# WarmCongee/SDUMC

Measured on AMD Instinct MI355X. Metric: train samples/sec at MOSEI feature shapes (two-stream forward + 6-term loss + backward + Adam), higher is better.
Workload: dtype f32

## Files before the change

### include/sdumc_hip.h

```cpp
#ifndef SDUMC_HIP_H
#define SDUMC_HIP_H

#include <stddef.h>
#include <stdint.h>

#ifdef __cplusplus
extern "C" {
#endif

#define SDUMC_OK 0
#define SDUMC_EINVAL (-1)
#define SDUMC_ELAUNCH (-2)
#define SDUMC_ENOMEM (-3)

#define SDUMC_MAX_GROUPS 8
#define SDUMC_D 256
#define SDUMC_H 128
#define SDUMC_NQ 7
#define SDUMC_RNC_DIM 64
#define SDUMC_N_SITES 35

typedef struct sdumc_dropout {
  uint32_t enabled;
  uint32_t site;
// ... 203 lines not shown
  size_t workspace_bytes;
  float* dq_sum;
  float* dout_masked;
} sdumc_attnpool_bwd_t;

size_t sdumc_attnpool_bwd_workspace_bytes(int32_t V, int32_t T, int32_t nq);
int sdumc_attnpool_bwd(const sdumc_attnpool_bwd_t* p, void* stream);
typedef struct sdumc_umca {
  sdumc_attnpool a;
  const float* w_in;
  const float* b_in;
  const void* x_p3;
  const void* w_in_p3f;
} sdumc_umca;
int sdumc_umca_fwd(const sdumc_umca* p, void* stream);

int sdumc_attnpool_fwd_multi(const sdumc_attnpool* sites, int32_t n, void* stream);
int sdumc_attnpool_bwd_multi(const sdumc_attnpool_bwd_t* sites, int32_t n, void* stream);
int sdumc_attnpool_set_v2_(int on);


int sdumc_relu_drop_bwd(const float* dy, const float* y, float scale, float* dz, int64_t n, void* stream);

size_t sdumc_colsum_workspace_bytes(int64_t rows, int32_t cols);
int sdumc_colsum(const float* a, int64_t rows, int32_t cols, int32_t lda, float* out, int32_t accumulate,
                 float* workspace, void* stream);

int sdumc_add_n(const float* const* xs, int32_t k, float* y, int64_t n, void* stream);

typedef struct sdumc_dropsum {
// ... 372 lines not shown
```

### sdumc_amd/_lib.py

```python
import ctypes as C
import os

_HERE = os.path.dirname(os.path.abspath(__file__))
LIB_PATH = os.environ.get("SDUMC_LIB") or os.path.join(_HERE, "csrc", "libsdumc_hip.so")

MAX_GROUPS = 8
D, H, NQ, RNC_DIM, N_SITES = 256, 128, 7, 64, 35
NT, NN, TN = 0, 1, 2
ACT_NONE, ACT_RELU, ACT_TANH = 0, 1, 2

c_float_p = C.c_void_p


class Dropout(C.Structure):
    _fields_ = [("enabled", C.c_uint32), ("site", C.c_uint32), ("threshold", C.c_uint32), ("scale", C.c_float),
                ("rows", C.c_uint32), ("width", C.c_uint32), ("samples", C.c_uint32), ("sample0", C.c_uint32),
                ("call0", C.c_uint32), ("stream0", C.c_uint32), ("seed_lo", C.c_uint32), ("seed_hi", C.c_uint32),
                ("dev_state", C.c_void_p), ("bits", C.c_void_p)]


class Gemm(C.Structure):
    _fields_ = [("layout", C.c_int32), ("M", C.c_int32), ("N", C.c_int32), ("K", C.c_int32),
                ("groups", C.c_int32),
                ("A", C.c_void_p * MAX_GROUPS), ("B", C.c_void_p * MAX_GROUPS),
# ... 266 lines not shown
    "sdumc_p3_join": (C.c_int, [C.c_void_p, C.c_int64, C.c_void_p, C.c_int64, C.c_int64, C.c_int32, C.c_void_p]),
    "sdumc_gemm_b1_workspace_bytes": (C.c_size_t, [C.POINTER(GemmB1)]),
    "sdumc_gemm_b1_nt": (C.c_int, [C.POINTER(GemmB1), C.c_void_p]),
    "sdumc_b1_frag_multi": (C.c_int, [C.c_void_p, C.c_void_p, C.POINTER(C.c_int64), C.POINTER(C.c_int64), C.POINTER(C.c_int32),
                                      C.POINTER(C.c_int32), C.c_int, C.c_void_p]),
    "sdumc_gemm_rows256": (C.c_int, [C.POINTER(RowsProblem), C.c_int32, C.c_void_p]),
    "sdumc_gemm_rows256_bf16": (C.c_int, [C.POINTER(RowsProblem), C.c_int32, C.c_void_p]),
    "sdumc_attnpool_fwd_workspace_bytes": (C.c_size_t, [C.c_int32, C.c_int32, C.c_int32]),
    "sdumc_attnpool_fwd": (C.c_int, [C.POINTER(AttnPool), C.c_void_p]),
    "sdumc_attnpool_fwd_workspace_bytes_dim": (C.c_size_t, [C.c_int32, C.c_int32, C.c_int32, C.c_int32]),
    "sdumc_attnpool_bwd_workspace_bytes_dim": (C.c_size_t, [C.c_int32, C.c_int32, C.c_int32, C.c_int32]),
    "sdumc_attnpool_bwd_workspace_bytes": (C.c_size_t, [C.c_int32, C.c_int32, C.c_int32]),
    "sdumc_attnpool_bwd": (C.c_int, [C.POINTER(AttnPoolBwd), C.c_void_p]),
    "sdumc_attnpool_fwd_multi": (C.c_int, [C.POINTER(AttnPool), C.c_int32, C.c_void_p]),
    "sdumc_umca_fwd": (C.c_int, [C.POINTER(Umca), C.c_void_p]),
    "sdumc_attnpool_bwd_multi": (C.c_int, [C.POINTER(AttnPoolBwd), C.c_int32, C.c_void_p]),
    "sdumc_relu_drop_bwd": (C.c_int, [C.c_void_p, C.c_void_p, C.c_float, C.c_void_p, C.c_int64, C.c_void_p]),
    "sdumc_colsum_workspace_bytes": (C.c_size_t, [C.c_int64, C.c_int32]),
    "sdumc_colsum": (C.c_int, [C.c_void_p, C.c_int64, C.c_int32, C.c_int32, C.c_void_p, C.c_int32, C.c_void_p, C.c_void_p]),
    "sdumc_add_n": (C.c_int, [C.POINTER(C.c_void_p), C.c_int32, C.c_void_p, C.c_int64, C.c_void_p]),
    "sdumc_dropsum_bwd": (C.c_int, [C.POINTER(DropSum), C.c_void_p]),
    "sdumc_fusion_fwd": (C.c_int, [C.c_void_p, C.c_void_p, C.c_void_p, C.c_int32, C.c_void_p]),
    "sdumc_fusion_bwd": (C.c_int, [C.c_void_p, C.c_void_p, C.c_void_p, C.c_void_p, C.c_void_p, C.c_int32, C.c_void_p]),
    "sdumc_hweight_fwd": (C.c_int, [C.c_void_p, C.c_void_p, C.c_void_p, C.c_int32, C.c_void_p]),
    "sdumc_hweight_bwd": (C.c_int, [C.c_void_p, C.c_void_p, C.c_void_p, C.c_void_p, C.c_void_p, C.c_void_p, C.c_int32, C.c_float, C.c_void_p]),
    "sdumc_zpool_fwd": (C.c_int, [C.c_void_p, C.c_void_p, C.c_void_p, C.c_int32, C.c_void_p]),
    "sdumc_zpool_bwd": (C.c_int, [C.c_void_p, C.c_void_p, C.c_void_p, C.c_void_p, C.c_void_p, C.c_int32, C.c_void_p]),
    "sdumc_mse_fwd_bwd": (C.c_int, [C.c_void_p, C.c_void_p, C.c_int32, C.c_float, C.c_float, C.c_void_p, C.c_void_p, C.c_void_p]),
    "sdumc_ssd_workspace_bytes": (C.c_size_t, [C.c_int64]),
    "sdumc_ssd": (C.c_int, [C.c_void_p, C.c_void_p, C.c_int64, C.c_void_p, C.c_void_p, C.c_void_p]),
# ... 153 lines not shown
```

### sdumc_amd/csrc/attn_pool.hip

```cpp
#include <type_traits>

#include "common.h"
#include "p3_loop.h"
#include <cstring>

namespace {

constexpr int D = SDUMC_D;
constexpr int MAXQ = 8;
constexpr int CH = 64;

__device__ __forceinline__ f32x4 ld4(const float* p) { return *reinterpret_cast<const f32x4*>(p); }
__device__ __forceinline__ void st4(float* p, f32x4 v) { *reinterpret_cast<f32x4*>(p) = v; }
__device__ __forceinline__ void stf_dev(float* p, float v) { __hip_atomic_store(p, v, __ATOMIC_RELAXED, __HIP_MEMORY_SCOPE_AGENT); }
__device__ __forceinline__ float ldf_dev(const float* p) { return __hip_atomic_load(p, __ATOMIC_RELAXED, __HIP_MEMORY_SCOPE_AGENT); }
__device__ __forceinline__ void st4_dev(float* p, f32x4 v) {
#pragma unroll
  for (int j = 0; j < 4; ++j) stf_dev(p + j, v[j]);
}
__device__ __forceinline__ f32x4 ld4_dev(const float* p) {
  f32x4 v;
#pragma unroll
  for (int j = 0; j < 4; ++j) v[j] = ldf_dev(p + j);
  return v;
// ... 114 lines not shown
    const size_t o = ((size_t)v * nq + i) * DD + 4 * cq;
    st4(p.pooled + o, sum);
    if (od.enabled) sum *= drop_mask4(od, (uint32_t)(v * nq + i), (uint32_t)cq);
    st4(p.out + o, sum);
  }
  float* attn = p.attn + (size_t)v * T * nq;
  for (int e = tid; e < T * nq; e += 256) {
    const int t = e / nq, i = e - t * nq;
    attn[e] = (DEV ? ldf_dev(attn + e) : attn[e]) * fac[(t / CH) * MAXQ + i];
  }
}

constexpr int UMCA_LDK = D + 4;
template <bool PHILOX, int C, bool HF = false, bool KLDS = false>
__device__ __forceinline__ void attn_fwd_partial_body(const sdumc_attnpool p, float* ws, const int nchunk, const int chunk, const int v,
                                                      const float* k_lds = nullptr, float* q_ext = nullptr, float* red_ext = nullptr) {
  constexpr int DD = D * C, LDQ = DD + 16;
  constexpr int RED = 4 * MAXQ * D > MAXQ * LDQ ? 4 * MAXQ * D : MAXQ * LDQ;
  __shared__ __attribute__((aligned(16))) float P_s[CH * MAXQ];
  float* red;
  if constexpr (KLDS) {
    red = red_ext;
  } else {
    __shared__ __attribute__((aligned(16))) float red_s[RED];
    red = red_s;
  }
  __shared__ float wstat[4][16];
  __shared__ float cstat[16];
  const int tid = threadIdx.x, lane = tid & 63, wave = tid >> 6;
  const int r16 = lane & 15, kk = lane >> 4;
  const int T = p.T, nq = p.nq;
  const int t0 = chunk * CH;
  const FwdWs w = fwd_ws(ws, p.V, nchunk, nq, DD);
  const bool fuse = p.tickets != nullptr;
  const int Tv = p.lengths ? min(T, max(1, p.lengths[v])) : T;

  float* q_s = KLDS ? q_ext : red;
  for (int e = tid; e < MAXQ * (DD / 4); e += 256) {
    const int i = e / (DD / 4), cq = e - i * (DD / 4);
    st4(q_s + i * LDQ + 4 * cq, i < nq ? ld4(p.q + (size_t)v * p.q_stride + (size_t)i * DD + 4 * cq) : f32x4{0.f, 0.f, 0.f, 0.f});
  }
  __syncthreads();
  constexpr int RB = 4;
  const DropRT xd = drop_resolve(p.x_drop);
// ... 1165 lines not shown
}
template <bool MASK>
__global__ __launch_bounds__(256, 2) void umca_fwd_kernel(const sdumc_umca u, const int nchunk) {
  extern __shared__ __attribute__((aligned(16))) char lds[];
  umca_fwd_body<MASK, false>(u, nchunk, lds);
}
template <bool MASK>
__global__ __launch_bounds__(256, 2) void umca_fwd_split_kernel(const sdumc_umca u, const int nchunk) {
  extern __shared__ __attribute__((aligned(16))) char lds[];
  umca_fwd_body<MASK, true>(u, nchunk, lds);
}

using K3P3Cfg_m = sdumc_p3::PCfg<64, 4, true, 4>;
using K3P3Cfg_n = sdumc_p3::PCfg<64, 4, false, 4>;
static_assert(K3P3Cfg_m::LDS_BYTES <= TOP_BYTES, "the P3 ring lies inside the key tile's memory");
template <bool MASK>
__global__ __launch_bounds__(256, 2) void umca_fwd_p3_kernel(const sdumc_umca u, const int nchunk) {
#if defined(__HIP_DEVICE_COMPILE__)
  using CF = std::conditional_t<MASK, K3P3Cfg_m, K3P3Cfg_n>;
  extern __shared__ __attribute__((aligned(16))) char lds[];
  const sdumc_attnpool& p = u.a;
  const int tid = threadIdx.x, lane = tid & 63;
  const int wave = __builtin_amdgcn_readfirstlane(tid >> 6);
  const int li = lane & 31, lh = lane >> 5;
  const int wn0 = wave * 64;
  const int chunk = blockIdx.x, v = blockIdx.y;
  const int T = p.T, t0 = chunk * CH, vx = v % p.x_samples;
  const __amdgpu_buffer_rsrc_t ra = __builtin_amdgcn_make_buffer_rsrc(const_cast<void*>(u.x_p3), 0,
      (int)min((size_t)p.x_samples * T * D * 6, (size_t)0xFFFFFFF0u), 0x00020000);
  const uint32_t qw = (p.x_drop.width + 3u) >> 2;
  const __amdgpu_buffer_rsrc_t rbits = __builtin_amdgcn_make_buffer_rsrc(const_cast<uint8_t*>(MASK ? p.x_drop.bits : static_cast<const uint8_t*>(u.x_p3)), 0,
      MASK ? (int)min((size_t)p.V * T * qw, (size_t)0xFFFFFFF0u) : 0, 0x00020000);
  f32x16 acc[2][2];
  sdumc_p3::p3_mainloop<CF>(lds, ra, (int64_t)D * 6, [&](int row) { return vx * T + min(t0 + row, T - 1); },
                            rbits, (int)qw, [&](int row) { return v * T + min(t0 + row, T - 1); },
                            static_cast<const char*>(u.w_in_p3f) + (size_t)(wave * 2) * (size_t)((D / 16) * sdumc_p3::FRAG_KT), (size_t)((D / 16) * sdumc_p3::FRAG_KT),
                            0, D / sdumc_p3::BK, acc);
  __syncthreads();
  const float mscale = MASK ? p.x_drop.scale : 1.f;
  float* K_s = reinterpret_cast<float*>(lds);
  float* q_s = reinterpret_cast<float*>(lds + TOP_BYTES);
  float* keys_out = const_cast<float*>(p.keys);
#pragma unroll
  for (int i = 0; i < 2; ++i)
#pragma unroll
    for (int j = 0; j < 2; ++j) {
      const int col = wn0 + 32 * j + li;
      const float bv = u.b_in[col];
#pragma unroll
      for (int e = 0; e < 16; ++e) {
        const int row = 32 * i + (e & 3) + 8 * (e >> 2) + 4 * lh;
        const float kv = fast_tanh(acc[i][j][e] * mscale + bv);
        K_s[row * UMCA_LDK + col] = kv;
        if (keys_out && t0 + row < T) keys_out[((size_t)v * T + t0 + row) * D + col] = kv;
      }
    }
  __syncthreads();
  attn_fwd_partial_body<false, 1, false, true>(p, static_cast<float*>(p.workspace), nchunk, chunk, v, K_s, q_s, K_s);
#endif
}

}

static inline uint32_t qw_of(const sdumc_dropout& d) { return (d.width + 3u) >> 2; }
extern "C" int sdumc_umca_fwd(const sdumc_umca* up, void* stream) {
  if (!up) return SDUMC_EINVAL;
  sdumc_umca u = *up;
  const sdumc_attnpool& p = u.a;
  if (p.V <= 0 || p.T <= 0 || p.nq < 1 || p.nq > MAXQ || p.x_samples <= 0) return SDUMC_EINVAL;
  if ((p.dim != 0 && p.dim != D) || p.bf16 || p.tickets) return SDUMC_EINVAL;
  if (!p.x || !p.q || !p.attn || !p.pooled || !p.out || !u.w_in || !u.b_in) return SDUMC_EINVAL;
  if (p.x_drop.enabled && !p.x_drop.bits) return SDUMC_EINVAL;
  if ((p.T + CH - 1) / CH > 4096) return SDUMC_EINVAL;
// ... 19 lines not shown
    if (p.x_drop.enabled) hipLaunchKernelGGL(sdumc_k3::umca_fwd_p3_kernel<true>, grid, blk, sdumc_k3::LDS_BYTES, st, u, nchunk);
    else hipLaunchKernelGGL(sdumc_k3::umca_fwd_p3_kernel<false>, grid, blk, sdumc_k3::LDS_BYTES, st, u, nchunk);
  } else if (sdumc_split_on_(SDUMC_SPLIT_UMCA)) {
    if (p.x_drop.enabled) hipLaunchKernelGGL(sdumc_k3::umca_fwd_split_kernel<true>, grid, blk, sdumc_k3::LDS_BYTES, st, u, nchunk);
    else hipLaunchKernelGGL(sdumc_k3::umca_fwd_split_kernel<false>, grid, blk, sdumc_k3::LDS_BYTES, st, u, nchunk);
  } else if (p.x_drop.enabled) hipLaunchKernelGGL(sdumc_k3::umca_fwd_kernel<true>, grid, blk, sdumc_k3::LDS_BYTES, st, u, nchunk);
  else hipLaunchKernelGGL(sdumc_k3::umca_fwd_kernel<false>, grid, blk, sdumc_k3::LDS_BYTES, st, u, nchunk);
  SDUMC_CHECK_LAUNCH();
  if (p.partial_only) return SDUMC_OK;
  hipLaunchKernelGGL(attn_fwd_combine_kernel, dim3(p.V), dim3(256), (size_t)nchunk * MAXQ * sizeof(float), st, p,
                     static_cast<const float*>(p.workspace), nchunk);
  SDUMC_CHECK_LAUNCH();
  return SDUMC_OK;
}

__global__ void sdumc_preload_attn_pool_kernel() {}
extern "C" int sdumc_preload_attn_pool_(void) {
  hipFuncAttributes a;
  return hipFuncGetAttributes(&a, reinterpret_cast<const void*>(&sdumc_preload_attn_pool_kernel)) == hipSuccess ? SDUMC_OK : SDUMC_ELAUNCH;
}
```

### sdumc_amd/csrc/common.h

```cpp
#pragma once
#include <hip/hip_runtime.h>
#include <stdint.h>
#include "../../include/sdumc_hip.h"

#define SDUMC_CHECK_LAUNCH()                                 \
  do {                                                       \
    if (hipGetLastError() != hipSuccess) return SDUMC_ELAUNCH; \
  } while (0)

typedef float f32x4 __attribute__((ext_vector_type(4)));
typedef float f32x16 __attribute__((ext_vector_type(16)));

static inline hipStream_t as_stream(void* s) { return (hipStream_t)s; }

#ifdef __cplusplus
#include <atomic>
#include <mutex>
struct sdumc_dev_once {
  std::mutex mu;
  std::atomic<uint64_t> done{0};
};
template <class F>
static inline int sdumc_once_per_device(sdumc_dev_once& o, F&& setup) {
  int dev = 0;
// ... 85 lines not shown
  uint32_t w[6];
};
int sdumc_dropout_bits_multi_ex_(const sdumc_dropout* d, int32_t streams, int32_t nsite, int32_t site_stride, uint8_t* const* bits,
                                 const uint32_t* tag, int32_t call_add, const struct sdumc_bits_shape* shape, void* stream);
int sdumc_bits_tag_(const sdumc_dropout* d, uint32_t* tag, int32_t call_add, const struct sdumc_bits_shape* shape, void* stream);
int sdumc_weights_to_bf16_(const float* src, void* dst, void* dst_t, const int64_t* offs, const int32_t* outs, const int32_t* ins,
                           const int32_t* want_t, int n, void* stream);
size_t sdumc_gg_slab_bytes_(int tiles);
int sdumc_gemm_rows_prepare_(void);
#define SDUMC_SPLIT_GROUP 1
#define SDUMC_SPLIT_WIDE 2
#define SDUMC_SPLIT_UMCA 4
#define SDUMC_SPLIT_ROWS 8
#define SDUMC_SPLIT_ALL 15
int sdumc_split_on_(int bit);
int sdumc_split_scope_(int mask);
int sdumc_gemm_rows256_capped_(const sdumc_rows_problem* probs, int32_t n, int32_t max_wg, void* stream);
int sdumc_gemm_rows256_bf16_capped_(const sdumc_rows_problem* probs, int32_t n, int32_t max_wg, void* stream);
int sdumc_p3_split_frag_multi_(const float* P, void* dst, const int64_t* src_off, const int64_t* dst_off, const int32_t* rows,
                               const int32_t* cols, int n, void* stream);
int sdumc_chain_transpose_(const float* src, float* dst, const int64_t* offs, const int32_t* outs, const int32_t* ins, int n,
                           void* stream);
struct sdumc_attn_layout {
  int32_t B, S;
  int32_t T[3][2];
  int64_t attn[2][3];
  int64_t total;
};
int sdumc_plan_attn_layout_(const sdumc_net_dims* d, struct sdumc_attn_layout* out);
}
// ... 99 lines not shown
```

### sdumc_amd/csrc/engine.hip

```cpp
#include <stdio.h>
#include <string.h>

#include <algorithm>
#include <atomic>
#include <map>
#include <cstdlib>
#include <cstring>
#include <mutex>
#include <string>
#include <tuple>
#include <vector>

#include "common.h"

extern "C" int sdumc_axpy2d(const float* src, int32_t ld_src, float* dst, int32_t ld_dst, int32_t rows, int32_t cols,
                            void* stream);

namespace {

constexpr int D = SDUMC_D, H = SDUMC_H, NQ = SDUMC_NQ, RD = SDUMC_RNC_DIM;

constexpr int SITE_IN[2][3] = {{0, 2, 4}, {21, 23, 25}};
constexpr int SITE_OUT[2][3] = {{1, 3, 5}, {22, 24, 26}};
constexpr int SITE_UMLP0 = 6, SITE_UMLP1 = 7;
// ... 1006 lines not shown
int p3_refresh_weights(const Ctx& c, int m) {
  const int din[3] = {c.d.da, c.d.dt, c.d.dv};
  int64_t so[3], dofs[3];
  int32_t rows[3], cols[3];
  so[0] = c.pm.frame[m].w; dofs[0] = c.pl.wp3_frame[m]; rows[0] = D; cols[0] = din[m];
  so[1] = c.pm.fra_proj[m].w; dofs[1] = c.pl.wp3_key[0][m]; rows[1] = D; cols[1] = D;
  so[2] = c.pm.ca_in[m].w; dofs[2] = c.pl.wp3_key[1][m]; rows[2] = D; cols[2] = D;
  return sdumc_p3_split_frag_multi_(c.P, wp3_ptr(c, 0), so, dofs, rows, cols, 3, c.st);
}
int feat_slot(int m, int s) { return m == 0 ? 0 : (m == 2 ? 2 : (s == 0 ? 1 : 3)); }
const int32_t* feat_map(const Ctx& c, int m, int s) { return c.io.row_map[feat_slot(m, s)]; }
int64_t feat_store_rows(const Ctx& c, int m, int s, bool both) {
  const int64_t a = c.io.store_rows[feat_slot(m, s)], b = both ? c.io.store_rows[feat_slot(m, 1)] : a;
  return (a > 0 && b > 0) ? std::max(a, b) : 0;
}
int p3_frame_proj(const Ctx& c, int m, int s, const void* feat_p3, int rows, int splitk, const void* feat2_p3 = nullptr, int rows2 = 0) {
  const int din[3] = {c.d.da, c.d.dt, c.d.dv};
  sdumc_gemm_p3 g;
  memset(&g, 0, sizeof(g));
  g.M = rows + rows2; g.N = D; g.K = din[m];
  g.A = feat_p3; g.lda = (int64_t)din[m] * 6;
  g.a_map = feat_map(c, m, s);
  g.a_map_rows = feat_store_rows(c, m, s, feat2_p3 != nullptr);
  if (feat2_p3) { g.A2 = feat2_p3; g.a2_row0 = rows; g.a2_map = feat_map(c, m, 1); }
  g.B = wp3_ptr(c, c.pl.wp3_frame[m]); g.ldb = (int64_t)(din[m] / 16) * 3072;
  g.bias = c.P + c.pm.frame[m].b;
  g.act = SDUMC_ACT_NONE;
  g.C = c.p(c.pl.x[m][s]); g.ldc = D;
  g.C_p3 = c.p(c.pl.xp3[m][s]); g.ldc_p3 = (int64_t)D * 6;
  g.splitk = splitk;
  g.workspace = c.scr;
  g.workspace_bytes = (size_t)c.pl.scratch_floats * sizeof(float);
  return sdumc_gemm_p3_nt(&g, c.st);
}
int p3_keys_fwd(const Ctx& c, int m, int k) {
  for (const Seg& sg : c.pl.segs[m]) {
    const Lin& L = k == 0 ? c.pm.fra_proj[m] : c.pm.ca_in[m];
    const sdumc_dropout dr = in_drop(c, k, m, sg.T, sg.s0, sg.row0);
    sdumc_gemm_p3 g;
    memset(&g, 0, sizeof(g));
    g.M = sg.V * sg.T; g.N = D; g.K = D;
    g.A = c.p(c.pl.xp3[m][sg.s0]); g.lda = (int64_t)D * 6;
    g.a_row_mod = sg.x_samples < sg.V ? sg.x_samples * sg.T : 0;
    if (dr.enabled) { g.a_bits = dr.bits; g.bits_qw = D / 4; g.a_scale = dr.scale; }
    g.B = wp3_ptr(c, c.pl.wp3_key[k][m]); g.ldb = (int64_t)(D / 16) * 3072;
    g.bias = c.P + L.b;
    g.act = SDUMC_ACT_TANH;
    g.C = c.p(c.pl.keys[k][m]) + sg.row0 * D; g.ldc = D;
    g.splitk = 1;
// ... 50 lines not shown
      a[n].workspace_bytes = bytes;
      ws += (bytes / sizeof(float) + 63) / 64 * 64;
      if (fra_fold(c)) fold_partial_only(c, k, order[oi], a[n]);
      ++n;
    }
  return sdumc_attnpool_fwd_multi(a, n, c.st);
}

bool k3_ok(const Ctx& c, int m) {
  static const int on = [] { const char* e = getenv("SDUMC_K3"); return e ? atoi(e) : 1; }();
  if (!on || c.h() || c.d.bf16) return false;
  for (const Seg& sg : c.pl.segs[m])
    if (sg.T < 96) return false;
  return true;
}
int umca_site(const Ctx& c, int k, int m, bool keep) {
  for (const Seg& sg : c.pl.segs[m]) {
    sdumc_umca u;
    memset(&u, 0, sizeof(u));
    u.a = attn_desc(c, k, m, sg);
    u.a.tickets = nullptr;
    if (!keep) u.a.keys = nullptr;
    u.a.workspace = c.scr;
    u.a.workspace_bytes = (size_t)c.pl.scratch_floats * sizeof(float);
    if (fra_fold(c)) fold_partial_only(c, k, m, u.a);
    const Lin& L = k == 0 ? c.pm.fra_proj[m] : c.pm.ca_in[m];
    u.w_in = c.P + L.w;
    u.b_in = c.P + L.b;
    if (p3_mode(c) && sdumc_split_on_(SDUMC_SPLIT_UMCA)) {
      u.x_p3 = c.p(c.pl.xp3[m][sg.s0]);
      u.w_in_p3f = wp3_ptr(c, c.pl.wp3_key[k][m]);
    }
    RET(sdumc_umca_fwd(&u, c.st));
  }
  return SDUMC_OK;
}

int pool_fwd(const Ctx& c, int k, int m) {
  for (const Seg& sg : c.pl.segs[m]) {
    sdumc_attnpool a = attn_desc(c, k, m, sg);
    a.workspace = c.scr;
    a.workspace_bytes = (size_t)c.pl.scratch_floats * sizeof(float);
    if (fra_fold(c)) fold_partial_only(c, k, m, a);
    RET(sdumc_attnpool_fwd(&a, c.st));
  }
  return SDUMC_OK;
}


bool use_chain(const Ctx& c) {
// ... 206 lines not shown
        if (hipEventRecord(bits_done[m], c.st) != hipSuccess) return SDUMC_ELAUNCH;
      }
    }
    if (pregen) {
      const sdumc_dropout d0 = mkdrop(c, SITE_IN[0][0], c.d.p_frame, pl.segs[0][0].T, D, 0);
      RET(sdumc_bits_tag_(&d0, reinterpret_cast<uint32_t*>(bits_set(c, 0)), 0, &shape_now, c.st));
    }
  }
  hipEvent_t fra_done[3] = {nullptr, nullptr, nullptr}, ca_done[3] = {nullptr, nullptr, nullptr};
  auto p3_frames = [&](int m) -> int {
    constexpr int p3_text_split = 4;
    RET(p3_refresh_weights(c, m));
    for (int s = 0; s < (m == 1 ? S : 1); ++s) {
      const void* fp = m == 0 ? c.io.audio_p3 : (m == 2 ? c.io.video_p3 : c.io.text_p3[s]);
      const int rows_p = B * pl.T[m][s];
      const bool few = rows_p < 8192 && din[m] >= 2048;
      if (m == 1 && S == 2 && few && rows_p % 64 == 0) {
        RET(p3_frame_proj(c, m, 0, fp, rows_p, p3_text_split, c.io.text_p3[1], B * pl.T[1][1]));
        break;
      }
      RET(p3_frame_proj(c, m, s, fp, rows_p, few ? 2 * p3_text_split : 1));
    }
    return SDUMC_OK;
  };
  for (int m = 0; m < 3; ++m) {
    c.use(LANE_OF[m]);
    if (p3_mode(c)) RET(p3_frames(m));
    if (b1_mode(c)) RET(b1_refresh_weights(c, m));
    for (int s = 0; s < (m == 1 ? S : 1) && !p3_mode(c); ++s) {
      const float* in = m == 0 ? c.io.audio : (m == 2 ? c.io.video : c.io.text[s]);
      if (b1_mode(c)) {
        const int rows_p = B * pl.T[m][s];
        if (m == 1 && S == 2 && rows_p % 64 == 0) {
          RET(b1_frame_proj(c, m, 0, in, rows_p, c.io.text[1], B * pl.T[1][1]));
          break;
        }
        RET(b1_frame_proj(c, m, s, in, rows_p));
        continue;
      }
      if (c.h()) {
        sdumc_gemm_bf16 g = GH_(SDUMC_NT, B * pl.T[m][s], D, din[m]);
        g.A[0] = in;
// ... 15 lines not shown
    }
    mark(c.st, 28 + 4 * m);
    if (bits_done[m] && hipStreamWaitEvent(c.st, bits_done[m], 0) != hipSuccess) return SDUMC_ELAUNCH;
    if (bits_with_xd) {
      for (const Seg& sg : pl.segs[m]) {
        const sdumc_dropout d = mkdrop(c, SITE_IN[0][m], c.d.p_frame, sg.T, D, sg.s0);
        uint8_t* bo[2] = {reinterpret_cast<uint8_t*>(c.p(pl.bits[0][m])) + sg.row0 * (D / 4),
                          reinterpret_cast<uint8_t*>(c.p(pl.bits[1][m])) + sg.row0 * (D / 4)};
        void* xo[2] = {c.ph(pl.xd[0][m], sg.row0 * D), c.ph(pl.xd[1][m], sg.row0 * D)};
        RET(sdumc_dropout_bits_apply_bf16(&d, sg.V / B, SITE_IN[1][m] - SITE_IN[0][m], bo, c.ph(sg.x_off), (int64_t)sg.x_samples * sg.T,
                                          xo, c.st));
      }
    }
    mark(c.st, 29 + 4 * m);
    const bool k3_site0 = k3_ok(c, m);
    constexpr int ca_own = 1;
    if (c.bg && (ca_own & (1 << m)) && LANE_OF[m] != 0 && c.multi && !c.capturing) {
      if (k3_site0) RET(umca_site(c, 0, m, true));
      else { RET(keys_gemm_fwd(c, m, 0, 1)); RET(pool_fwd(c, 0, m)); }
      fra_done[m] = next_event(c);
      if (hipEventRecord(fra_done[m], c.st) != hipSuccess) return SDUMC_ELAUNCH;
      RET(keys_gemm_fwd(c, m, 1, 2));
      ca_done[m] = next_event(c);
      if (hipEventRecord(ca_done[m], c.st) != hipSuccess) return SDUMC_ELAUNCH;
    } else if (c.bg) {
      if (k3_site0) RET(umca_site(c, 0, m, true));
      else RET(keys_gemm_fwd(c, m, 0, 1));
      RET(link(c, LANE_OF[m], 3));
      c.use(3);
      RET(keys_gemm_fwd(c, m, 1, 2));
      c.use(LANE_OF[m]);
      if (!k3_site0) RET(pool_fwd(c, 0, m));
    } else if (k3_site0) {
      RET(umca_site(c, 0, m, true));
      RET(keys_gemm_fwd(c, m, 1, 2));
    } else {
      RET(keys_gemm_fwd(c, m, 0, 2));
      RET(pool_fwd(c, 0, m));
    }
    mark(c.st, 30 + 4 * m);
  }
  mark(c.sts[3], 40);
  c.use(0);
  for (int lane = 1; lane <= 2; ++lane) {
    int m_of = -1;
    for (int m = 0; m < 3; ++m) if (LANE_OF[m] == lane && fra_done[m]) m_of = m;
    if (m_of >= 0) {
      if (hipStreamWaitEvent(c.sts[0], fra_done[m_of], 0) != hipSuccess) return SDUMC_ELAUNCH;
    } else {
// ... 1212 lines not shown
```

### sdumc_amd/csrc/gemm_f32.hip

```cpp
#include <algorithm>
#include <cstring>
#include <mutex>
#include <type_traits>
#include <vector>

#include "common.h"

namespace {

struct ProfRec {
  hipEvent_t a, b;
  int variant;
  double flops;
};
bool g_prof_on = false;
std::vector<ProfRec> g_prof;
std::mutex g_prof_mu;
constexpr int kNumVariants = 29;
const char* const kVariantName[kNumVariants] = {"gemm_nt_128x128", "gemm_nt_64x64",  "gemm_nn_128x128",
                                                "gemm_nn_64x64",   "gemm_tn_128x128", "gemm_tn_64x64",
                                                "gemm_small_nt",   "gemm_small_nn",   "gemm_small_tn",
                                                "gemm_bf16_nt_128x128", "gemm_bf16_nt_64x64",
                                                "gemm_bf16_nn_128x128", "gemm_bf16_nn_64x64",
                                                "gemm_bf16_tn_128x128", "gemm_bf16_tn_64x64",
                                                "gemm_wide_nt", "gemm_wide_tn",
                                                "gemm_bf16s_nt", "gemm_bf16s_tn",
                                                "gemm_group_tn", "gemm_group_tn_bf16",
                                                "gemm_rows256", "gemm_rows256_bf16",
                                                "gemm_wide_nt_bf16x3", "gemm_group_tn_bf16x3", "gemm_rows256_bf16x3",
                                                "gemm_p3_nt_bf16x3", "gemm_p3_nt_masked_bf16x3",
                                                "gemm_b1_nt_bf16"};

constexpr int BK = 32;
constexpr int LDK = BK + 4;
#ifndef SDUMC_GEMM_WPE128
#define SDUMC_GEMM_WPE128 2
#endif
#ifndef SDUMC_GEMM_WPE64
#define SDUMC_GEMM_WPE64 5
#endif

struct TileLoadCtx {
  const float* p;
  int ld;
  int row_mod;
  bool vec;
// ... 901 lines not shown
```

### sdumc_amd/csrc/p3_loop.h

```cpp
#pragma once
#include <type_traits>

#include "common.h"

namespace sdumc_p3 {

typedef __attribute__((address_space(3))) void lds_void_t;
typedef __attribute__((address_space(1))) const void gbl_void_t;
typedef const __attribute__((address_space(4))) int32_t const_i32_t;
typedef __bf16 bf16x8 __attribute__((ext_vector_type(8)));
typedef __bf16 bf16x2 __attribute__((ext_vector_type(2)));
typedef float f32x2s __attribute__((ext_vector_type(2)));
typedef uint32_t u32x4 __attribute__((ext_vector_type(4)));

constexpr int waitcnt_vm(int n) { return (n & 0xF) | ((n >> 4) << 14) | (0x7 << 4) | (0xF << 8); }

__device__ __forceinline__ float fast_tanh(float x) { return 1.f - 2.f * __frcp_rn(1.f + __expf(2.f * x)); }

__device__ __forceinline__ uint32_t pk(float x, float y) {
  const f32x2s v = {x, y};
  return __builtin_bit_cast(uint32_t, __builtin_convertvector(v, bf16x2));
}
__device__ __forceinline__ void split8(const float (&v)[8], u32x4 (&pl)[3]) {
#pragma unroll
// ... 25 lines not shown
  static constexpr int BITS_LDS = MASK ? BITS_P * 256 : 0;
  static constexpr int STAGE = A_BYTES + BITS_LDS;
  static constexpr int LDT = 32 * TN + 4;
  static constexpr int EPI_BYTES = NW * 32 * LDT * 4;
  static constexpr int LDS_BYTES = NST * STAGE > EPI_BYTES ? NST * STAGE : EPI_BYTES;
  static_assert(BM % 32 == 0 && A_BYTES % 1024 == 0 && NA <= 2 && (NW == 4 || NW == 8), "tile shape");
  static_assert(BITS_P <= NW, "one keep-bits piece per wave");
  static_assert(NST >= DB + 1, "the A stage a step needs must be older in the queue than the B fragments it needs");
  static_assert(3 * (3 * TN + NA + 1) < 64, "vmcnt is a 6-bit counter");
};

template <class CF, class SrcRow, class BitsRow>
__device__ __forceinline__ void p3_mainloop(char* lds, const __amdgpu_buffer_rsrc_t ra, const int64_t lda, SrcRow src_row,
                                            const __amdgpu_buffer_rsrc_t rbits, const int bits_qw, BitsRow bits_row, const char* bwave,
                                            const size_t bblk, const int kbeg, const int nk, f32x16 (&acc)[CF::TM][CF::TN],
                                            uint64_t* stamp = nullptr) {
#if defined(__HIP_DEVICE_COMPILE__)
  constexpr int NST = CF::NST, TM = CF::TM, TN = CF::TN, NW = CF::NW;
  constexpr bool MASK = CF::MASK;
  const int tid = threadIdx.x, lane = tid & 63;
  const int wave = __builtin_amdgcn_readfirstlane(tid >> 6);
  const int li = lane & 31, lh = lane >> 5;
  constexpr bool GA = std::is_pointer<decltype(src_row(0))>::value;
  [[maybe_unused]] uint32_t voff[CF::NA];
  [[maybe_unused]] const char* gaddr[CF::NA];
  bool pvalid[CF::NA];
#pragma unroll
  for (int i = 0; i < CF::NA; ++i) {
    const int piece = wave + i * NW;
    pvalid[i] = piece < CF::A_P;
    const int q = (min(piece, CF::A_P - 1) << 6) + lane;
    const int row = q / 6, sl = q - 6 * row;
    const int hp = sl >= 3 ? 1 : 0, p = sl - 3 * hp;
    const int h = hp ^ ((row >> 3) & 1);
    if constexpr (GA) gaddr[i] = reinterpret_cast<const char*>(src_row(row)) + (size_t)((kbeg >> 3) + h) * 48u + (size_t)p * 16u;
// ... 165 lines not shown
```

Baseline: 50140.

## Fuse frame projection GEMM with UMCA attention-pool forward into one kernel

Adds a kernel that first computes the per-frame input projection (bf16x3 P3 GEMM plus bias), writing both the f32 and the split-bf16 copies. In the same workgroup it then runs the UMCA key-projection and attention-pool partial body for one or both streams. This replaces a separate frame-projection GEMM launch followed by the UMCA launch, saving one kernel launch and letting the second stage read its input while it is likely still in cache. It is on by default for eligible modalities (not text, single segment, not in graph capture) and can be turned off with an env var. The costs are a heavier kernel that reloads kernel arguments to limit register pressure, and less parallelism between the two stages.

```diff
diff --git a/include/sdumc_hip.h b/include/sdumc_hip.h
--- a/include/sdumc_hip.h
+++ b/include/sdumc_hip.h
@@ -241,6 +241,8 @@
   const void* w_in_p3f;
 } sdumc_umca;
 int sdumc_umca_fwd(const sdumc_umca* p, void* stream);
+int sdumc_frame_umca_fwd_p3(const sdumc_gemm_p3* g, const sdumc_umca* u, void* stream);
+int sdumc_set_frame_k3(int on);
 
 int sdumc_attnpool_fwd_multi(const sdumc_attnpool* sites, int32_t n, void* stream);
 int sdumc_attnpool_bwd_multi(const sdumc_attnpool_bwd_t* sites, int32_t n, void* stream);
diff --git a/sdumc_amd/_lib.py b/sdumc_amd/_lib.py
--- a/sdumc_amd/_lib.py
+++ b/sdumc_amd/_lib.py
@@ -304,6 +304,8 @@
     "sdumc_attnpool_bwd": (C.c_int, [C.POINTER(AttnPoolBwd), C.c_void_p]),
     "sdumc_attnpool_fwd_multi": (C.c_int, [C.POINTER(AttnPool), C.c_int32, C.c_void_p]),
     "sdumc_umca_fwd": (C.c_int, [C.POINTER(Umca), C.c_void_p]),
+    "sdumc_frame_umca_fwd_p3": (C.c_int, [C.POINTER(GemmP3), C.POINTER(Umca), C.c_void_p]),
+    "sdumc_set_frame_k3": (C.c_int, [C.c_int]),
     "sdumc_attnpool_bwd_multi": (C.c_int, [C.POINTER(AttnPoolBwd), C.c_int32, C.c_void_p]),
     "sdumc_relu_drop_bwd": (C.c_int, [C.c_void_p, C.c_void_p, C.c_float, C.c_void_p, C.c_int64, C.c_void_p]),
     "sdumc_colsum_workspace_bytes": (C.c_size_t, [C.c_int64, C.c_int32]),
diff --git a/sdumc_amd/csrc/attn_pool.hip b/sdumc_amd/csrc/attn_pool.hip
--- a/sdumc_amd/csrc/attn_pool.hip
+++ b/sdumc_amd/csrc/attn_pool.hip
@@ -2,6 +2,8 @@
 
 #include "common.h"
 #include "p3_loop.h"
+#include <atomic>
+#include <cstdlib>
 #include <cstring>
 
 namespace {
@@ -152,7 +154,8 @@
 constexpr int UMCA_LDK = D + 4;
 template <bool PHILOX, int C, bool HF = false, bool KLDS = false>
 __device__ __forceinline__ void attn_fwd_partial_body(const sdumc_attnpool p, float* ws, const int nchunk, const int chunk, const int v,
-                                                      const float* k_lds = nullptr, float* q_ext = nullptr, float* red_ext = nullptr) {
+                                                      const float* k_lds = nullptr, float* q_ext = nullptr, float* red_ext = nullptr,
+                                                      const int tid_in = threadIdx.x) {
   constexpr int DD = D * C, LDQ = DD + 16;
   constexpr int RED = 4 * MAXQ * D > MAXQ * LDQ ? 4 * MAXQ * D : MAXQ * LDQ;
   __shared__ __attribute__((aligned(16))) float P_s[CH * MAXQ];
@@ -165,7 +168,7 @@
   }
   __shared__ float wstat[4][16];
   __shared__ float cstat[16];
-  const int tid = threadIdx.x, lane = tid & 63, wave = tid >> 6;
+  const int tid = tid_in, lane = tid & 63, wave = tid >> 6;
   const int r16 = lane & 15, kk = lane >> 4;
   const int T = p.T, nq = p.nq;
   const int t0 = chunk * CH;
@@ -1361,17 +1364,17 @@
 using K3P3Cfg_m = sdumc_p3::PCfg<64, 4, true, 4>;
 using K3P3Cfg_n = sdumc_p3::PCfg<64, 4, false, 4>;
 static_assert(K3P3Cfg_m::LDS_BYTES <= TOP_BYTES, "the P3 ring lies inside the key tile's memory");
-template <bool MASK>
-__global__ __launch_bounds__(256, 2) void umca_fwd_p3_kernel(const sdumc_umca u, const int nchunk) {
+template <bool MASK, bool FRESH = false>
+__device__ __forceinline__ void umca_fwd_p3_body(const sdumc_umca& u, const int nchunk, char* lds, const int chunk, const int v) {
 #if defined(__HIP_DEVICE_COMPILE__)
   using CF = std::conditional_t<MASK, K3P3Cfg_m, K3P3Cfg_n>;
-  extern __shared__ __attribute__((aligned(16))) char lds[];
   const sdumc_attnpool& p = u.a;
-  const int tid = threadIdx.x, lane = tid & 63;
+  int tid = threadIdx.x;
+  if constexpr (FRESH) asm volatile("" : "+v"(tid));
+  const int lane = tid & 63;
   const int wave = __builtin_amdgcn_readfirstlane(tid >> 6);
   const int li = lane & 31, lh = lane >> 5;
   const int wn0 = wave * 64;
-  const int chunk = blockIdx.x, v = blockIdx.y;
   const int T = p.T, t0 = chunk * CH, vx = v % p.x_samples;
   const __amdgpu_buffer_rsrc_t ra = __builtin_amdgcn_make_buffer_rsrc(const_cast<void*>(u.x_p3), 0,
       (int)min((size_t)p.x_samples * T * D * 6, (size_t)0xFFFFFFF0u), 0x00020000);
@@ -1382,7 +1385,7 @@
   sdumc_p3::p3_mainloop<CF>(lds, ra, (int64_t)D * 6, [&](int row) { return vx * T + min(t0 + row, T - 1); },
                             rbits, (int)qw, [&](int row) { return v * T + min(t0 + row, T - 1); },
                             static_cast<const char*>(u.w_in_p3f) + (size_t)(wave * 2) * (size_t)((D / 16) * sdumc_p3::FRAG_KT), (size_t)((D / 16) * sdumc_p3::FRAG_KT),
-                            0, D / sdumc_p3::BK, acc);
+                            0, D / sdumc_p3::BK, acc, nullptr, tid);
   __syncthreads();
   const float mscale = MASK ? p.x_drop.scale : 1.f;
   float* K_s = reinterpret_cast<float*>(lds);
@@ -1403,7 +1406,105 @@
       }
     }
   __syncthreads();
-  attn_fwd_partial_body<false, 1, false, true>(p, static_cast<float*>(p.workspace), nchunk, chunk, v, K_s, q_s, K_s);
+  attn_fwd_partial_body<false, 1, false, true>(p, static_cast<float*>(p.workspace), nchunk, chunk, v, K_s, q_s, K_s, tid);
+#endif
+}
+template <bool MASK>
+__global__ __launch_bounds__(256, 2) void umca_fwd_p3_kernel(const sdumc_umca u, const int nchunk) {
+  extern __shared__ __attribute__((aligned(16))) char lds[];
+  umca_fwd_p3_body<MASK>(u, nchunk, lds, blockIdx.x, blockIdx.y);
+}
+
+using FrameCfg = sdumc_p3::PCfg<64, 4, false, 4>;
+static_assert(FrameCfg::LDS_BYTES <= TOP_BYTES, "the projection's ring and staging lie inside the key tile's memory");
+struct FrameUmcaArgs {
+  sdumc_gemm_p3 g;
+  sdumc_umca u;
+  int nchunk, nstream;
+};
+template <class A>
+__device__ __forceinline__ A fresh_kernarg() {
+  typedef const __attribute__((address_space(4))) uint32_t kword_t;
+  kword_t* kw = (kword_t*)__builtin_amdgcn_kernarg_segment_ptr();
+  asm volatile("" : "+s"(kw));
+  uint32_t w[sizeof(A) / 4];
+#pragma unroll
+  for (int i = 0; i < (int)(sizeof(A) / 4); ++i) w[i] = kw[i];
+  A r;
+  __builtin_memcpy(&r, w, sizeof(A));
+  return r;
+}
+template <bool MASK>
+__global__ __launch_bounds__(256, 2) void frame_umca_fwd_p3_kernel(const FrameUmcaArgs a) {
+#if defined(__HIP_DEVICE_COMPILE__)
+  using CF = FrameCfg;
+  using sdumc_p3::split8;
+  using sdumc_p3::u32x4;
+  extern __shared__ __attribute__((aligned(16))) char lds[];
+  const sdumc_gemm_p3& g = a.g;
+  const int tid = threadIdx.x, lane = tid & 63;
+  const int wave = __builtin_amdgcn_readfirstlane(tid >> 6);
+  const int li = lane & 31, lh = lane >> 5;
+  const int chunk = blockIdx.x, vx = blockIdx.y;
+  const int T = a.u.a.T, t0 = chunk * CH;
+  {
+    constexpr int TM = CF::TM, TN = CF::TN;
+    const __amdgpu_buffer_rsrc_t ra = __builtin_amdgcn_make_buffer_rsrc(const_cast<void*>(g.A), 0, (int)min((size_t)g.M * (size_t)g.lda, (size_t)0xFFFFFFF0u), 0x00020000);
+    const __amdgpu_buffer_rsrc_t rnone = __builtin_amdgcn_make_buffer_rsrc(const_cast<void*>(g.A), 0, 0, 0x00020000);
+    f32x16 acc[TM][TN];
+    sdumc_p3::p3_mainloop<CF>(lds, ra, g.lda, [&](int row) { return vx * T + min(t0 + row, T - 1); }, rnone, 0, [&](int) { return 0; },
+                              static_cast<const char*>(g.B) + (size_t)(wave * TN) * (size_t)g.ldb, (size_t)g.ldb, 0, g.K / sdumc_p3::BK, acc);
+    constexpr int LDT = CF::LDT, WCOLS = 32 * TN, CPW = WCOLS / 8;
+    float* tw = reinterpret_cast<float*>(lds) + wave * 32 * LDT;
+    const int colw = WCOLS * wave;
+    float bv[8];
+#pragma unroll
+    for (int c = 0; c < 8; ++c) bv[c] = g.bias ? g.bias[colw + 8 * (lane & (CPW - 1)) + c] : 0.f;
+    __syncthreads();
+#pragma unroll
+    for (int i = 0; i < TM; ++i) {
+#pragma unroll
+      for (int j = 0; j < TN; ++j)
+#pragma unroll
+        for (int e = 0; e < 16; ++e) tw[((e & 3) + 8 * (e >> 2) + 4 * lh) * LDT + 32 * j + li] = acc[i][j][e];
+      __builtin_amdgcn_s_waitcnt(0xC07F);
+#pragma unroll
+      for (int u = lane; u < 32 * CPW; u += 64) {
+        const int r = u / CPW, cq = u % CPW;
+        const int t = t0 + 32 * i + r, col = colw + 8 * cq;
+        if (t < T) {
+          const size_t row = (size_t)vx * T + t;
+          const f32x4 a0 = *reinterpret_cast<const f32x4*>(tw + r * LDT + 8 * cq), a1 = *reinterpret_cast<const f32x4*>(tw + r * LDT + 8 * cq + 4);
+          float v[8] = {a0[0], a0[1], a0[2], a0[3], a1[0], a1[1], a1[2], a1[3]};
+#pragma unroll
+          for (int c = 0; c < 8; ++c) v[c] = v[c] + bv[c];
+          float* dst = g.C + row * g.ldc + col;
+          *reinterpret_cast<f32x4*>(dst) = f32x4{v[0], v[1], v[2], v[3]};
+          *reinterpret_cast<f32x4*>(dst + 4) = f32x4{v[4], v[5], v[6], v[7]};
+          u32x4 pl[3];
+          split8(v, pl);
+          char* dp = static_cast<char*>(g.C_p3) + row * (size_t)g.ldc_p3 + (size_t)(col >> 3) * 48;
+          *reinterpret_cast<u32x4*>(dp) = pl[0];
+          *reinterpret_cast<u32x4*>(dp + 16) = pl[1];
+          *reinterpret_cast<u32x4*>(dp + 32) = pl[2];
+        }
+      }
+      __builtin_amdgcn_s_waitcnt(0xC07F);
+    }
+  }
+  __builtin_amdgcn_s_waitcnt(0);
+  __syncthreads();
+  auto site = [&](auto second) {
+    const FrameUmcaArgs a2 = fresh_kernarg<FrameUmcaArgs>();
+    int ch2 = chunk, vx2 = vx;
+    asm volatile("" : "+s"(ch2), "+s"(vx2));
+    umca_fwd_p3_body<MASK, true>(a2.u, a2.nchunk, lds, ch2, (decltype(second)::value ? a2.u.a.x_samples : 0) + vx2);
+  };
+  site(std::false_type{});
+  if (a.nstream > 1) {
+    __syncthreads();
+    site(std::true_type{});
+  }
 #endif
 }
 
@@ -1453,6 +1554,69 @@
   return SDUMC_OK;
 }
 
+extern "C" int sdumc_prof_begin_(int variant, double flops, void* stream);
+extern "C" void sdumc_prof_end_(int token, void* stream);
+
+namespace { std::atomic<int> g_frame_k3_on{-1}; }
+extern "C" int sdumc_set_frame_k3(int on) {
+  g_frame_k3_on.store(on ? 1 : 0);
+  return SDUMC_OK;
+}
+extern "C" int sdumc_frame_k3_on_(void) {
+  if (g_frame_k3_on.load() < 0) { const char* e = getenv("SDUMC_FRAME_K3"); g_frame_k3_on.store(e ? (atoi(e) ? 1 : 0) : 1); }
+  return g_frame_k3_on.load();
+}
+
+extern "C" int sdumc_frame_umca_fwd_p3(const sdumc_gemm_p3* gp, const sdumc_umca* up, void* stream) {
+  using namespace sdumc_p3;
+  if (!gp || !up) return SDUMC_EINVAL;
+  const sdumc_gemm_p3& g = *gp;
+  sdumc_umca u = *up;
+  const sdumc_attnpool& p = u.a;
+  if (g.M <= 0 || g.N != BN || g.K <= 0 || (g.K % (4 * BK))) return SDUMC_EINVAL;
+  if (!g.A || !g.B || !g.C || !g.C_p3) return SDUMC_EINVAL;
+  if ((reinterpret_cast<uintptr_t>(g.A) | reinterpret_cast<uintptr_t>(g.B) | reinterpret_cast<uintptr_t>(g.C) | reinterpret_cast<uintptr_t>(g.C_p3)) & 15) return SDUMC_EINVAL;
+  if (g.lda < 6 * (int64_t)g.K || (g.lda & 15)) return SDUMC_EINVAL;
+  if (g.ldb < (int64_t)(g.K / BK) * FRAG_KT || (g.ldb & 15)) return SDUMC_EINVAL;
+  if (g.act != SDUMC_ACT_NONE || g.tile_m != 0 || g.splitk > 1) return SDUMC_EINVAL;
+  if (g.a_map || g.a2_map || g.A2 || g.a_row_mod || g.a_bits) return SDUMC_EINVAL;
+  if ((size_t)g.M * (size_t)g.lda >= 0xFFFFFFF0u) return SDUMC_EINVAL;
+  if (p.V <= 0 || p.T <= 0 || p.nq < 1 || p.nq > MAXQ || p.x_samples <= 0) return SDUMC_EINVAL;
+  if (p.V != p.x_samples && p.V != 2 * p.x_samples) return SDUMC_EINVAL;
+  if ((p.dim != 0 && p.dim != D) || p.bf16 || p.tickets) return SDUMC_EINVAL;
+  if (!p.x || !p.q || !p.attn || !p.pooled || !p.out || !u.w_in || !u.b_in || !u.x_p3 || !u.w_in_p3f) return SDUMC_EINVAL;
+  if (p.x_drop.enabled && !p.x_drop.bits) return SDUMC_EINVAL;
+  if ((p.T + CH - 1) / CH > 4096) return SDUMC_EINVAL;
+  if (!sdumc_split_on_(SDUMC_SPLIT_UMCA)) return SDUMC_EINVAL;
+  if ((reinterpret_cast<uintptr_t>(u.x_p3) | reinterpret_cast<uintptr_t>(u.w_in_p3f)) & 15) return SDUMC_EINVAL;
+  if (p.x_drop.enabled && (qw_of(p.x_drop) & 3)) return SDUMC_EINVAL;
+  if (g.M != p.x_samples * p.T || g.C != p.x || g.C_p3 != u.x_p3 || g.ldc != D || g.ldc_p3 != (int64_t)D * 6) return SDUMC_EINVAL;
+  if (!p.workspace || p.workspace_bytes < sdumc_attnpool_fwd_workspace_bytes_dim(p.V, p.T, p.nq, D)) return SDUMC_ENOMEM;
+  static sdumc_dev_once attr;
+  if (sdumc_once_per_device(attr, [] {
+        return sdumc_set_dyn_lds(&sdumc_k3::frame_umca_fwd_p3_kernel<true>, sdumc_k3::LDS_BYTES) &&
+               sdumc_set_dyn_lds(&sdumc_k3::frame_umca_fwd_p3_kernel<false>, sdumc_k3::LDS_BYTES);
+      }) != SDUMC_OK)
+    return SDUMC_ELAUNCH;
+  hipStream_t st = as_stream(stream);
+  sdumc_k3::FrameUmcaArgs a;
+  a.g = g;
+  a.u = u;
+  a.nchunk = (p.T + CH - 1) / CH;
+  a.nstream = p.V / p.x_samples;
+  const dim3 grid(a.nchunk, p.x_samples), blk(256);
+  const int tok = sdumc_prof_begin_(29, 2.0 * g.M * (double)g.N * g.K + 2.0 * p.V * (double)p.T * D * D, stream);
+  if (p.x_drop.enabled) hipLaunchKernelGGL(sdumc_k3::frame_umca_fwd_p3_kernel<true>, grid, blk, sdumc_k3::LDS_BYTES, st, a);
+  else hipLaunchKernelGGL(sdumc_k3::frame_umca_fwd_p3_kernel<false>, grid, blk, sdumc_k3::LDS_BYTES, st, a);
+  SDUMC_CHECK_LAUNCH();
+  sdumc_prof_end_(tok, stream);
+  if (p.partial_only) return SDUMC_OK;
+  hipLaunchKernelGGL(attn_fwd_combine_kernel, dim3(p.V), dim3(256), (size_t)a.nchunk * MAXQ * sizeof(float), st, p,
+                     static_cast<const float*>(p.workspace), a.nchunk);
+  SDUMC_CHECK_LAUNCH();
+  return SDUMC_OK;
+}
+
 __global__ void sdumc_preload_attn_pool_kernel() {}
 extern "C" int sdumc_preload_attn_pool_(void) {
   hipFuncAttributes a;
diff --git a/sdumc_amd/csrc/common.h b/sdumc_amd/csrc/common.h
--- a/sdumc_amd/csrc/common.h
+++ b/sdumc_amd/csrc/common.h
@@ -123,6 +123,7 @@
 #define SDUMC_SPLIT_ROWS 8
 #define SDUMC_SPLIT_ALL 15
 int sdumc_split_on_(int bit);
+int sdumc_frame_k3_on_(void);
 int sdumc_split_scope_(int mask);
 int sdumc_gemm_rows256_capped_(const sdumc_rows_problem* probs, int32_t n, int32_t max_wg, void* stream);
 int sdumc_gemm_rows256_bf16_capped_(const sdumc_rows_problem* probs, int32_t n, int32_t max_wg, void* stream);
diff --git a/sdumc_amd/csrc/engine.hip b/sdumc_amd/csrc/engine.hip
--- a/sdumc_amd/csrc/engine.hip
+++ b/sdumc_amd/csrc/engine.hip
@@ -1044,7 +1044,7 @@
   const int64_t a = c.io.store_rows[feat_slot(m, s)], b = both ? c.io.store_rows[feat_slot(m, 1)] : a;
   return (a > 0 && b > 0) ? std::max(a, b) : 0;
 }
-int p3_frame_proj(const Ctx& c, int m, int s, const void* feat_p3, int rows, int splitk, const void* feat2_p3 = nullptr, int rows2 = 0) {
+sdumc_gemm_p3 p3_frame_desc(const Ctx& c, int m, int s, const void* feat_p3, int rows, int splitk, const void* feat2_p3 = nullptr, int rows2 = 0) {
   const int din[3] = {c.d.da, c.d.dt, c.d.dv};
   sdumc_gemm_p3 g;
   memset(&g, 0, sizeof(g));
@@ -1061,8 +1061,13 @@
   g.splitk = splitk;
   g.workspace = c.scr;
   g.workspace_bytes = (size_t)c.pl.scratch_floats * sizeof(float);
+  return g;
+}
+int p3_frame_proj(const Ctx& c, int m, int s, const void* feat_p3, int rows, int splitk, const void* feat2_p3 = nullptr, int rows2 = 0) {
+  const sdumc_gemm_p3 g = p3_frame_desc(c, m, s, feat_p3, rows, splitk, feat2_p3, rows2);
   return sdumc_gemm_p3_nt(&g, c.st);
 }
+bool p3_few_rows(int rows, int din) { return rows < 8192 && din >= 2048; }
 int p3_keys_fwd(const Ctx& c, int m, int k) {
   for (const Seg& sg : c.pl.segs[m]) {
     const Lin& L = k == 0 ? c.pm.fra_proj[m] : c.pm.ca_in[m];
@@ -1143,26 +1148,44 @@
     if (sg.T < 96) return false;
   return true;
 }
+sdumc_umca umca_desc(const Ctx& c, int k, int m, const Seg& sg, bool keep) {
+  sdumc_umca u;
+  memset(&u, 0, sizeof(u));
+  u.a = attn_desc(c, k, m, sg);
+  u.a.tickets = nullptr;
+  if (!keep) u.a.keys = nullptr;
+  u.a.workspace = c.scr;
+  u.a.workspace_bytes = (size_t)c.pl.scratch_floats * sizeof(float);
+  if (fra_fold(c)) fold_partial_only(c, k, m, u.a);
+  const Lin& L = k == 0 ? c.pm.fra_proj[m] : c.pm.ca_in[m];
+  u.w_in = c.P + L.w;
+  u.b_in = c.P + L.b;
+  if (p3_mode(c) && sdumc_split_on_(SDUMC_SPLIT_UMCA)) {
+    u.x_p3 = c.p(c.pl.xp3[m][sg.s0]);
+    u.w_in_p3f = wp3_ptr(c, c.pl.wp3_key[k][m]);
+  }
+  return u;
+}
 int umca_site(const Ctx& c, int k, int m, bool keep) {
   for (const Seg& sg : c.pl.segs[m]) {
-    sdumc_umca u;
-    memset(&u, 0, sizeof(u));
-    u.a = attn_desc(c, k, m, sg);
-    u.a.tickets = nullptr;
-    if (!keep) u.a.keys = nullptr;
-    u.a.workspace = c.scr;
-    u.a.workspace_bytes = (size_t)c.pl.scratch_floats * sizeof(float);
-    if (fra_fold(c)) fold_partial_only(c, k, m, u.a);
-    const Lin& L = k == 0 ? c.pm.fra_proj[m] : c.pm.ca_in[m];
-    u.w_in = c.P + L.w;
-    u.b_in = c.P + L.b;
-    if (p3_mode(c) && sdumc_split_on_(SDUMC_SPLIT_UMCA)) {
-      u.x_p3 = c.p(c.pl.xp3[m][sg.s0]);
-      u.w_in_p3f = wp3_ptr(c, c.pl.wp3_key[k][m]);
-    }
+    const sdumc_umca u = umca_desc(c, k, m, sg, keep);
     RET(sdumc_umca_fwd(&u, c.st));
   }
   return SDUMC_OK;
+}
+bool frame_k3_ok(const Ctx& c, int m) {
+  if (!sdumc_frame_k3_on_() || c.capturing || !p3_mode(c) || !k3_ok(c, m) || !sdumc_split_on_(SDUMC_SPLIT_UMCA)) return false;
+  if (m == 1 || feat_map(c, m, 0) || c.pl.segs[m].size() != 1) return false;
+  const int din[3] = {c.d.da, c.d.dt, c.d.dv};
+  const Seg& sg = c.pl.segs[m][0];
+  return sg.s0 == 0 && !p3_few_rows(sg.x_samples * sg.T, din[m]);
+}
+int frame_umca_site(const Ctx& c, int m) {
+  const Seg& sg = c.pl.segs[m][0];
+  const void* fp = m == 0 ? c.io.audio_p3 : (m == 2 ? c.io.video_p3 : c.io.text_p3[0]);
+  const sdumc_gemm_p3 g = p3_frame_desc(c, m, 0, fp, sg.x_samples * sg.T, 1);
+  const sdumc_umca u = umca_desc(c, 0, m, sg, true);
+  return sdumc_frame_umca_fwd_p3(&g, &u, c.st);
 }
 
 int pool_fwd(const Ctx& c, int k, int m) {
@@ -1399,7 +1422,7 @@
     for (int s = 0; s < (m == 1 ? S : 1); ++s) {
       const void* fp = m == 0 ? c.io.audio_p3 : (m == 2 ? c.io.video_p3 : c.io.text_p3[s]);
       const int rows_p = B * pl.T[m][s];
-      const bool few = rows_p < 8192 && din[m] >= 2048;
+      const bool few = p3_few_rows(rows_p, din[m]);
       if (m == 1 && S == 2 && few && rows_p % 64 == 0) {
         RET(p3_frame_proj(c, m, 0, fp, rows_p, p3_text_split, c.io.text_p3[1], B * pl.T[1][1]));
         break;
@@ -1410,7 +1433,9 @@
   };
   for (int m = 0; m < 3; ++m) {
     c.use(LANE_OF[m]);
-    if (p3_mode(c)) RET(p3_frames(m));
+    const bool fused = frame_k3_ok(c, m);
+    if (fused) RET(p3_refresh_weights(c, m));
+    else if (p3_mode(c)) RET(p3_frames(m));
     if (b1_mode(c)) RET(b1_refresh_weights(c, m));
     for (int s = 0; s < (m == 1 ? S : 1) && !p3_mode(c); ++s) {
       const float* in = m == 0 ? c.io.audio : (m == 2 ? c.io.video : c.io.text[s]);
@@ -1456,9 +1481,10 @@
     }
     mark(c.st, 29 + 4 * m);
     const bool k3_site0 = k3_ok(c, m);
+    auto k3_site = [&]() -> int { return fused ? frame_umca_site(c, m) : umca_site(c, 0, m, true); };
     constexpr int ca_own = 1;
     if (c.bg && (ca_own & (1 << m)) && LANE_OF[m] != 0 && c.multi && !c.capturing) {
-      if (k3_site0) RET(umca_site(c, 0, m, true));
+      if (k3_site0) RET(k3_site());
       else { RET(keys_gemm_fwd(c, m, 0, 1)); RET(pool_fwd(c, 0, m)); }
       fra_done[m] = next_event(c);
       if (hipEventRecord(fra_done[m], c.st) != hipSuccess) return SDUMC_ELAUNCH;
@@ -1466,7 +1492,7 @@
       ca_done[m] = next_event(c);
       if (hipEventRecord(ca_done[m], c.st) != hipSuccess) return SDUMC_ELAUNCH;
     } else if (c.bg) {
-      if (k3_site0) RET(umca_site(c, 0, m, true));
+      if (k3_site0) RET(k3_site());
       else RET(keys_gemm_fwd(c, m, 0, 1));
       RET(link(c, LANE_OF[m], 3));
       c.use(3);
@@ -1474,7 +1500,7 @@
       c.use(LANE_OF[m]);
       if (!k3_site0) RET(pool_fwd(c, 0, m));
     } else if (k3_site0) {
-      RET(umca_site(c, 0, m, true));
+      RET(k3_site());
       RET(keys_gemm_fwd(c, m, 1, 2));
     } else {
       RET(keys_gemm_fwd(c, m, 0, 2));
diff --git a/sdumc_amd/csrc/gemm_f32.hip b/sdumc_amd/csrc/gemm_f32.hip
--- a/sdumc_amd/csrc/gemm_f32.hip
+++ b/sdumc_amd/csrc/gemm_f32.hip
@@ -16,7 +16,7 @@
 bool g_prof_on = false;
 std::vector<ProfRec> g_prof;
 std::mutex g_prof_mu;
-constexpr int kNumVariants = 29;
+constexpr int kNumVariants = 30;
 const char* const kVariantName[kNumVariants] = {"gemm_nt_128x128", "gemm_nt_64x64",  "gemm_nn_128x128",
                                                 "gemm_nn_64x64",   "gemm_tn_128x128", "gemm_tn_64x64",
                                                 "gemm_small_nt",   "gemm_small_nn",   "gemm_small_tn",
@@ -29,7 +29,8 @@
                                                 "gemm_rows256", "gemm_rows256_bf16",
                                                 "gemm_wide_nt_bf16x3", "gemm_group_tn_bf16x3", "gemm_rows256_bf16x3",
                                                 "gemm_p3_nt_bf16x3", "gemm_p3_nt_masked_bf16x3",
-                                                "gemm_b1_nt_bf16"};
+                                                "gemm_b1_nt_bf16",
+                                                "frame_umca_fwd_p3_bf16x3"};
 
 constexpr int BK = 32;
 constexpr int LDK = BK + 4;
diff --git a/sdumc_amd/csrc/p3_loop.h b/sdumc_amd/csrc/p3_loop.h
--- a/sdumc_amd/csrc/p3_loop.h
+++ b/sdumc_amd/csrc/p3_loop.h
@@ -63,11 +63,11 @@
 __device__ __forceinline__ void p3_mainloop(char* lds, const __amdgpu_buffer_rsrc_t ra, const int64_t lda, SrcRow src_row,
                                             const __amdgpu_buffer_rsrc_t rbits, const int bits_qw, BitsRow bits_row, const char* bwave,
                                             const size_t bblk, const int kbeg, const int nk, f32x16 (&acc)[CF::TM][CF::TN],
-                                            uint64_t* stamp = nullptr) {
+                                            uint64_t* stamp = nullptr, const int tid_in = threadIdx.x) {
 #if defined(__HIP_DEVICE_COMPILE__)
   constexpr int NST = CF::NST, TM = CF::TM, TN = CF::TN, NW = CF::NW;
   constexpr bool MASK = CF::MASK;
-  const int tid = threadIdx.x, lane = tid & 63;
+  const int tid = tid_in, lane = tid & 63;
   const int wave = __builtin_amdgcn_readfirstlane(tid >> 6);
   const int li = lane & 31, lh = lane >> 5;
   constexpr bool GA = std::is_pointer<decltype(src_row(0))>::value;
```

After: 48370. 0.965x the previous value.
